# wusize/CLIPSelf

Measured on AMD Instinct MI355X. Metric: images/sec (student+teacher distill step), ViT-B/16 32 crops/img, higher is better.
Workload: dtype bf16; 1 GPU; EVA02-CLIP-B-16 CLIPSelf image-patches step, 64 images x 32 crops per GPU, 224^2 (BASELINE configs[1]); global_batch=64, crops_per_image=32, image_size=224, parallelism=dp1, teacher_chunk=2048, teacher_last_block=cls_query_only, teacher_schedule=one_batch_ahead_on_side_stream

## Files before the change

clipself_amd/csrc/attention.hip:

```cpp
#include <type_traits>
#include "cs_common.h"
#include <cstdlib>

namespace {

constexpr int HD = 64;
constexpr float LOG2E = 1.4426950408889634f;


#define Z16 (f32x16{0.f, 0.f, 0.f, 0.f, 0.f, 0.f, 0.f, 0.f, 0.f, 0.f, 0.f, 0.f, 0.f, 0.f, 0.f, 0.f})
__device__ __forceinline__ f32x16 zero16() {
    f32x16 z;
#pragma unroll
    for (int e = 0; e < 16; ++e) z[e] = 0.f;
    return z;
}

__device__ __forceinline__ void rope8(U128& v, const float* __restrict__ cs, const float* __restrict__ sn) {
    const float4 c0 = *(const float4*)cs, c1 = *(const float4*)(cs + 4);
    const float4 s0 = *(const float4*)sn, s1 = *(const float4*)(sn + 4);
    const float c[8] = {c0.x, c0.y, c0.z, c0.w, c1.x, c1.y, c1.z, c1.w};
    const float s[8] = {s0.x, s0.y, s0.z, s0.w, s1.x, s1.y, s1.z, s1.w};
#pragma unroll
    for (int j = 0; j < 4; ++j) {
        const float x0 = bf2f(v.e[2 * j]), x1 = bf2f(v.e[2 * j + 1]);
        v.e[2 * j] = f2bf(__builtin_fmaf(x0, c[2 * j], -(x1 * s[2 * j])));
        v.e[2 * j + 1] = f2bf(__builtin_fmaf(x1, c[2 * j + 1], x0 * s[2 * j + 1]));
    }
}

__device__ __forceinline__ void rope8_lds(U128& v, const float* rt, int g, float inv_g, int tok, int c8) {
    const int t = tok - 1;
    const int r = (int)(((float)t + 0.5f) * inv_g), c = t - r * g;
    const float* cs = rt + ((c8 < 4 ? r : 2 * g + c) << 5) + (c8 & 3) * 8;
    rope8(v, cs, cs + (g << 5));
}

template <int NT>
__device__ __forceinline__ void load_rope_tables(float* rt, const float* __restrict__ cos_t, const float* __restrict__ sin_t, int g, int tid) {
    for (int i = tid; i < g * 32; i += NT) {
        const int r = i >> 5, d = i & 31;
        rt[i] = cos_t[(size_t)(r * g) * HD + d];
        rt[(g << 5) + i] = sin_t[(size_t)(r * g) * HD + d];
        rt[(2 * g << 5) + i] = cos_t[(size_t)r * HD + 32 + d];
        rt[(3 * g << 5) + i] = sin_t[(size_t)r * HD + 32 + d];
    }
}

__device__ __forceinline__ bf16x8 pack8(const f32x16& a, int c2) {
    bf16x8 r;
#pragma unroll
    for (int j = 0; j < 8; ++j) r[j] = f2bf(a[c2 * 8 + j]);
    return r;
}

__device__ __forceinline__ bf16x8 load_t_frag(const __bf16* t, int ld, int d, int base, int hf) {
    U64 lo, hi;
    lo.u = *(const uint2*)(t + d * ld + base + 4 * hf);
    hi.u = *(const uint2*)(t + d * ld + base + 8 + 4 * hf);
    bf16x8 r;
#pragma unroll
    for (int j = 0; j < 4; ++j) { r[j] = lo.e[j]; r[4 + j] = hi.e[j]; }
    return r;
}

#ifdef CS_ABLATION_SWITCHES
#define ATT_ABL(p, bit) ((p).dbg & (bit))
#else
#define ATT_ABL(p, bit) false
#endif
struct AttnArgs {
    const __bf16* qkv;
    const __bf16* dout;
    const float* cos_t;
    const float* sin_t;
    const float* lse_in;
    const float* dsum;
    int dbg;
    int grid;
    float inv_grid;
    float* stats_part;
    long Mtot;
    __bf16* out;
    float* lse_out;
    int Ntok, H, ldqkv, ldo;
    float scale;
    int sch_on, sch_f0, sch_r, sch_bh, sch_fb, sch_rem, sch_absorb;
    const __bf16* qk;
    int ldqk;
};

struct RowBlock { int bh, tile0, nt; };
__device__ __forceinline__ RowBlock map_block(const AttnArgs& p, int waves) {
    RowBlock r;
    if (!p.sch_on) {
        r.bh = blockIdx.y; r.tile0 = blockIdx.x * waves; r.nt = waves;
        return r;
    }
    const int id = blockIdx.x;
    if (id < p.sch_f0) {
        const int qb = id / p.sch_bh;
        r.bh = id - qb * p.sch_bh; r.tile0 = qb * 8; r.nt = 8;
    } else if (id < p.sch_f0 + 2 * p.sch_r) {
        const int j = id - p.sch_f0, k = p.sch_f0 + (j >> 1), half = j & 1, qb = k / p.sch_bh;
        r.bh = k - qb * p.sch_bh; r.tile0 = qb * 8 + half * 4;
        r.nt = 4 + ((p.sch_absorb && half && qb == p.sch_fb - 1) ? p.sch_rem : 0);
    } else {
        r.bh = id - p.sch_f0 - 2 * p.sch_r; r.tile0 = p.sch_fb * 8; r.nt = p.sch_rem;
    }
    return r;
}

template <int CHK, bool ROPE, bool WITH_T>
__device__ __forceinline__ void stage_rows(const __bf16* __restrict__ src, size_t rowbase, int ld, int coloff, int tok0, int Ntok,
                                           const float* cos_t, const float* sin_t, char* tile, __bf16* tile_t, int ldt, int tid) {
    for (int idx = tid; idx < CHK * 8; idx += 512) {
        const int r = idx >> 3, c = idx & 7, tok = tok0 + r;
        U128 v;
        if (tok < Ntok) {
            v.u = *(const uint4*)(src + (rowbase + tok) * ld + coloff + c * 8);
            if (ROPE && tok > 0) rope8(v, cos_t + (size_t)(tok - 1) * HD + c * 8, sin_t + (size_t)(tok - 1) * HD + c * 8);
        } else {
            v.u = make_uint4(0, 0, 0, 0);
        }
        if (tile) *(uint4*)(tile + r * 128 + ((c ^ (r & 7)) << 4)) = v.u;
        if (WITH_T) {
#pragma unroll
            for (int e = 0; e < 8; ++e) tile_t[(c * 8 + e) * ldt + r] = v.e[e];
        }
    }
}

__device__ __forceinline__ bf16x8 lds_frag(const char* tile, int row, int ks, int hf) {
    return *(const bf16x8*)(tile + row * 128 + ((((ks << 1) + hf) ^ (row & 7)) << 4));
}

constexpr int VT_LD = 264;

__device__ __forceinline__ int k_off(int r, int c) { return ((r >> 1) << 8) + (((((r & 1) << 3) | c) ^ ((r >> 1) & 15)) << 4); }

typedef short s16x4v __attribute__((ext_vector_type(4)));

__device__ __forceinline__ int tr_lane_off(int rr, int d0, int lane) {
    const int li = lane & 15, g1 = (lane >> 4) & 1;
    const int col = d0 + 16 * g1 + 4 * (li & 3);
    return k_off(rr + (li >> 2), col >> 3) + ((col >> 2) & 1) * 8;
}
__device__ __forceinline__ bf16x8 tr_join2(s16x4v lo, s16x4v hi) {
    typedef short s16x8v __attribute__((ext_vector_type(8)));
    const s16x8v v = __builtin_shufflevector(lo, hi, 0, 1, 2, 3, 4, 5, 6, 7);
    return __builtin_bit_cast(bf16x8, v);
}
__device__ __forceinline__ s16x4v tr_read4(const char* addr) {
    return __builtin_amdgcn_ds_read_tr16_b64_v4i16((__attribute__((address_space(3))) s16x4v*)addr);
}

// ... 653 lines not shown
    {
        U128 t[4];
#pragma unroll
        for (int ks = 0; ks < 4; ++ks) {
            t[ks].u = PRE ? *(const uint4*)(p.qk + (rowbase + kc) * p.ldqk + C + h * HD + ks * 16 + hf * 8)
                          : *(const uint4*)(p.qkv + (rowbase + kc) * p.ldqkv + C + h * HD + ks * 16 + hf * 8);
            vf[ks] = *(const bf16x8*)(p.qkv + (rowbase + kc) * p.ldqkv + 2 * C + h * HD + ks * 16 + hf * 8);
        }
#pragma unroll
        for (int ks = 0; ks < 4; ++ks) {
            if (!PRE && ROPE && kc > 0) rope8_lds(t[ks], rt, p.grid, p.inv_grid, kc, ks * 2 + hf);
            kf[ks] = t[ks].h;
        }
    }
    f32x16 dk[2] = {zero16(), zero16()}, dv[2] = {zero16(), zero16()};
    const int k_base = (l31 >> 1) << 8, par8 = (l31 & 1) << 3, sw = l31 >> 1;
    int toff[2][2][2];
#pragma unroll
    for (int c2 = 0; c2 < 2; ++c2)
#pragma unroll
        for (int dt = 0; dt < 2; ++dt) {
            toff[c2][dt][0] = tr_lane_off(c2 * 16 + 4 * hf, dt * 32, lane);
            toff[c2][dt][1] = tr_lane_off(c2 * 16 + 8 + 4 * hf, dt * 32, lane);
        }

    for (int q0 = 0; q0 < (SINGLE ? 1 : p.Ntok); q0 += CHQ) {
        if (q0) __syncthreads();
        qr.template store<!PRE && ROPE>(Ql, rt, p.grid, p.inv_grid, q0, p.Ntok, tid);
        gr.template store<false>(Gl, rt, p.grid, p.inv_grid, q0, p.Ntok, tid);
        if (tid < CHQ) { lse_s[tid] = lse_r; dsum_s[tid] = dsum_r; }
        __syncthreads();
        if (!SINGLE && PF && q0 + CHQ < p.Ntok) {
            qr.load(qsrc, rowbase, qld, h * HD, q0 + CHQ, p.Ntok, tid);
            gr.load(p.dout, rowbase, p.ldo, h * HD, q0 + CHQ, p.Ntok, tid);
            load_stats(q0 + CHQ);
        }
        auto tile = [&](int t) {
            f32x16 s, dp;
#pragma unroll
            for (int ks = 0; ks < 4; ++ks) {
                const int off = t * (16 * 256) + k_base + (((par8 | (ks * 2 + hf)) ^ sw) << 4);
                s = __builtin_amdgcn_mfma_f32_32x32x16_bf16(*(const bf16x8*)(Ql + off), kf[ks], ks ? s : Z16, 0, 0, 0);
                dp = __builtin_amdgcn_mfma_f32_32x32x16_bf16(*(const bf16x8*)(Gl + off), vf[ks], ks ? dp : Z16, 0, 0, 0);
            }
#pragma unroll
            for (int k4 = 0; k4 < 4; ++k4) {
                const float4 l4 = *(const float4*)(lse_s + t * 32 + 8 * k4 + 4 * hf), d4 = *(const float4*)(dsum_s + t * 32 + 8 * k4 + 4 * hf);
                const float ls[4] = {l4.x, l4.y, l4.z, l4.w}, ds[4] = {d4.x, d4.y, d4.z, d4.w};
#pragma unroll
                for (int r = 0; r < 4; ++r) {
                    const int e = k4 * 4 + r;
                    const float pv = __builtin_amdgcn_exp2f(fmaf(s[e], sl2, -ls[r]));
                    s[e] = pv;
                    dp[e] = pv * fmaf(dp[e], p.scale, -ds[r]);
                }
            }
#pragma unroll
            for (int c2 = 0; c2 < 2; ++c2) {
                const bf16x8 pb = pack8(s, c2), db = pack8(dp, c2);
#pragma unroll
                for (int dt = 0; dt < 2; ++dt) {
                    const int o0 = t * (16 * 256) + toff[c2][dt][0], o1 = t * (16 * 256) + toff[c2][dt][1];
                    dv[dt] = __builtin_amdgcn_mfma_f32_32x32x16_bf16(tr_join2(tr_read4(Gl + o0), tr_read4(Gl + o1)), pb, dv[dt], 0, 0, 0);
                    dk[dt] = __builtin_amdgcn_mfma_f32_32x32x16_bf16(tr_join2(tr_read4(Ql + o0), tr_read4(Ql + o1)), db, dk[dt], 0, 0, 0);
                }
            }
        };
        if (wave_active) {
#pragma unroll
            for (int t = 0; t < CH; ++t) {
                if (q0 + t * 32 >= p.Ntok) break;
                tile(t);
            }
        }
    }
    if (wave_active && key < p.Ntok) {
        const size_t pos = (size_t)(key > 0 ? key - 1 : 0) * HD;
        __bf16* row = p.out + (rowbase + key) * p.ldqkv + h * HD;
        store_grad_tile(dk, row + C, ROPE && key > 0, p.cos_t + pos, p.sin_t + pos, hf);
        store_grad_tile(dv, row + 2 * C, false, nullptr, nullptr, hf);
    }
}

int att_num_cus() {
    static const int n = [] {
        int dev = 0, v = 0;
        if (hipGetDevice(&dev) != hipSuccess || hipDeviceGetAttribute(&v, hipDeviceAttributeMultiprocessorCount, dev) != hipSuccess || v <= 0) v = 256;
        return v;
    }();
    return n;
}
int set_schedule(AttnArgs& a, int B, int Ntok, int H, dim3& grid) {
    const int nt = (Ntok + 31) / 32, fb = nt / 8, rem = nt % 8, BH = B * H, F = fb * BH, G = att_num_cus();
    int R = F % G;
    if (getenv("CS_ATTN_NOSPLIT") || fb == 0 || 2 * R > G) R = 0;
    if (R == 0) {
        a.sch_on = 0;
        grid = dim3((Ntok + 255) / 256, BH);
        return 0;
    }
    a.sch_on = 1; a.sch_f0 = F - R; a.sch_r = R; a.sch_bh = BH; a.sch_fb = fb; a.sch_rem = rem;
    a.sch_absorb = rem > 0 && rem <= 4 && R >= BH;
    grid = dim3(F + R + ((rem > 0 && !a.sch_absorb) ? BH : 0), 1);
    return 1;
}

template <typename K>
void set_lds(K kernel, size_t bytes) { (void)hipFuncSetAttribute((const void*)kernel, hipFuncAttributeMaxDynamicSharedMemorySize, (int)bytes); }

int check_common(const char* who, int B, int Ntok, int H, int ldqkv, int ldo) {
    CS_CHECK_ARG(B > 0 && Ntok > 1 && H > 0, "%s: bad shape B=%d N=%d H=%d", who, B, Ntok, H);
    CS_CHECK_ARG(ldqkv % 8 == 0 && ldo % 8 == 0 && ldqkv >= 3 * H * HD && ldo >= H * HD, "%s: bad leading dimensions", who);
    return 0;
}

int check_tables(const char* who, const float* cos_t, const float* sin_t) {
    CS_CHECK_ARG((cos_t == nullptr) == (sin_t == nullptr), "%s: cos_t and sin_t are given together, or both NULL (no rotary embedding); got %s only",
                 who, cos_t ? "cos_t" : "sin_t");
    return 0;
}

template <int HG>
__global__ __launch_bounds__(256) void attn_cls_kernel(const __bf16* __restrict__ q, const __bf16* __restrict__ kv,
                                                       const float* __restrict__ cos_t, const float* __restrict__ sin_t,
                                                       __bf16* __restrict__ out, int Ntok, int H, int ldq, int ldkv, int ldo, float scale,
                                                       int qpb, const unsigned char* __restrict__ allow, float* __restrict__ lse_out) {
    extern __shared__ float sm[];
    const int Npad = (Ntok + 3) & ~3;
    float* rsum = sm + HG * Npad;
    float* part = rsum + 8;
    const int tid = threadIdx.x, lane = tid & 63, wave = tid >> 6;
    const int b = blockIdx.x, h0 = blockIdx.y * HG;
    const int c = tid & 7, kg = tid >> 3;
    const __bf16* kbase = kv + (size_t)(b / qpb) * Ntok * ldkv + h0 * HD + c * 8;
    const unsigned char* arow = allow ? allow + (size_t)b * Ntok : nullptr;
    const __bf16* vbase = kbase + H * HD;
    float qf[HG][8];
#pragma unroll
    for (int h = 0; h < HG; ++h) {
        U128 t;
        t.u = *(const uint4*)(q + (size_t)b * ldq + (h0 + h) * HD + c * 8);
#pragma unroll
        for (int j = 0; j < 8; ++j) qf[h][j] = bf2f(t.e[j]);
    }
    const float sl2 = scale * LOG2E;
    for (int key = kg; key < Ntok; key += 32) {
        U128 kk[HG];
#pragma unroll
        for (int h = 0; h < HG; ++h) kk[h].u = *(const uint4*)(kbase + (size_t)key * ldkv + h * HD);
        if (key > 0 && cos_t) {
            const float* cs = cos_t + (size_t)(key - 1) * HD + c * 8;
            const float* sn = sin_t + (size_t)(key - 1) * HD + c * 8;
#pragma unroll
            for (int h = 0; h < HG; ++h) rope8(kk[h], cs, sn);
        }
#pragma unroll
        for (int h = 0; h < HG; ++h) {
            float dot = 0.f;
#pragma unroll
            for (int j = 0; j < 8; ++j) dot += qf[h][j] * bf2f(kk[h].e[j]);
            dot += __shfl_xor(dot, 1);
            dot += __shfl_xor(dot, 2);
            dot += __shfl_xor(dot, 4);
            if (c == 0) sm[h * Npad + key] = (arow && !arow[key]) ? -INFINITY : dot * sl2;
        }
    }
    __syncthreads();
    for (int h = wave; h < HG; h += 4) {
        float* row = sm + h * Npad;
        float mx = -INFINITY;
        for (int key = lane; key < Ntok; key += 64) mx = fmaxf(mx, row[key]);
        mx = wave_max(mx);
        const bool no_key = mx == -INFINITY;
        if (no_key) mx = 0.f;
        float sum = 0.f;
        for (int key = lane; key < Ntok; key += 64) {
            const float e = __builtin_amdgcn_exp2f(row[key] - mx);
            sum += e;
            row[key] = bf2f(f2bf(e));
        }
        sum = wave_sum(sum);
        if (lane == 0) rsum[h] = sum > 0.f ? sum : 1.f;
        if (lane == 0 && lse_out)
            lse_out[((size_t)(b / qpb) * H + h0 + h) * qpb + b % qpb] = no_key ? INFINITY : (mx + __builtin_log2f(sum)) * (1.f / LOG2E);
    }
    __syncthreads();
    float acc[HG][8];
// ... 320 lines not shown
}

}

static int attn_fwd_impl(const void* qkv, const float* cos_t, const float* sin_t, void* out, float* lse, float* stats_part, int B, int Ntok,
                         int H, int ldqkv, int ldo, float scale, hipStream_t stream) {
    if (check_common("cs_attn_fwd", B, Ntok, H, ldqkv, ldo) || check_tables("cs_attn_fwd", cos_t, sin_t)) return -1;
    const bool rope = cos_t != nullptr;
    AttnArgs a{};
    a.qkv = (const __bf16*)qkv; a.cos_t = cos_t; a.sin_t = sin_t; a.out = (__bf16*)out; a.lse_out = lse;
    a.stats_part = stats_part; a.Mtot = (long)B * Ntok;
    int g = 0;
    if (rope) {
        g = (int)(sqrtf((float)(Ntok - 1)) + 0.5f);
        CS_CHECK_ARG(g * g == Ntok - 1, "cs_attn_fwd: Ntok - 1 = %d is not a square token grid (the RoPE tables are read separably)", Ntok - 1);
        a.grid = g; a.inv_grid = 1.f / (float)g;
    }
#ifdef CS_ABLATION_SWITCHES
    static const int dbg_env = getenv("CS_ATTN_DBG") ? atoi(getenv("CS_ATTN_DBG")) : 0;
    a.dbg = dbg_env;
#else
    a.dbg = 0;
#endif
    a.Ntok = Ntok; a.H = H; a.ldqkv = ldqkv; a.ldo = ldo; a.scale = scale;
    constexpr int CH = 7;
    const size_t lds = (size_t)CH * 32 * 128 + (size_t)HD * VT_LD * 2 + (size_t)4 * g * 32 * sizeof(float);
    CS_CHECK_ARG(lds <= 160 * 1024, "cs_attn_fwd: token grid %d too large for the LDS RoPE tables", g);
    if (Ntok <= CH * 32) {
        static bool once = (set_lds(attn_fwd8_kernel<false>, 160 * 1024), set_lds(attn_fwd8_kernel<true>, 160 * 1024),
                            set_lds(attn_fwd8_kernel<false, false>, 160 * 1024), set_lds(attn_fwd8_kernel<true, false>, 160 * 1024), true);
        (void)once;
        const bool tail = Ntok > (CH - 1) * 32;
        if (rope) {
            if (tail) hipLaunchKernelGGL((attn_fwd8_kernel<true>), dim3(1, B * H), dim3(512), lds, stream, a);
            else hipLaunchKernelGGL((attn_fwd8_kernel<false>), dim3(1, B * H), dim3(512), lds, stream, a);
        } else {
            if (tail) hipLaunchKernelGGL((attn_fwd8_kernel<true, false>), dim3(1, B * H), dim3(512), lds, stream, a);
            else hipLaunchKernelGGL((attn_fwd8_kernel<false, false>), dim3(1, B * H), dim3(512), lds, stream, a);
        }
    } else {
        static bool once = (set_lds(attn_fwd2_kernel<CH, 4>, 160 * 1024), set_lds(attn_fwd2_kernel<CH, 4, false>, 160 * 1024), true);
        (void)once;
        const size_t lds2 = (size_t)2 * CH * 32 * 128 + (size_t)4 * g * 32 * sizeof(float);
        dim3 grid2;
        set_schedule(a, B, Ntok, H, grid2);
        if (rope) hipLaunchKernelGGL((attn_fwd2_kernel<CH, 4>), grid2, dim3(512), lds2, stream, a);
        else hipLaunchKernelGGL((attn_fwd2_kernel<CH, 4, false>), grid2, dim3(512), lds2, stream, a);
    }
    CS_LAUNCH_CHECK();
    return 0;
}

extern "C" int cs_attn_fwd(const void* qkv, const float* cos_t, const float* sin_t, void* out, float* lse, int B, int Ntok, int H,
                           int ldqkv, int ldo, float scale, hipStream_t stream) {
    return attn_fwd_impl(qkv, cos_t, sin_t, out, lse, nullptr, B, Ntok, H, ldqkv, ldo, scale, stream);
}

extern "C" int cs_attn_fwd_stats(const void* qkv, const float* cos_t, const float* sin_t, void* out, float* lse, float* stats_part, int B,
                                 int Ntok, int H, int ldqkv, int ldo, float scale, hipStream_t stream) {
    CS_CHECK_ARG(stats_part != nullptr && ((uintptr_t)stats_part % 8) == 0, "cs_attn_fwd_stats: stats_part must be an 8-byte aligned buffer");
    return attn_fwd_impl(qkv, cos_t, sin_t, out, lse, stats_part, B, Ntok, H, ldqkv, ldo, scale, stream);
}

static size_t bwd_dsum_bytes(int B, int Ntok, int H) { return (((size_t)B * H * Ntok * sizeof(float)) + 255) & ~(size_t)255; }
static size_t bwd_image_bytes(int B, int Ntok, int H) {
    return bwd_dsum_bytes(B, Ntok, H) + (Ntok > 7 * 32 ? (size_t)B * Ntok * 2 * H * HD * sizeof(__bf16) : 0);
}
extern "C" size_t cs_attn_bwd_workspace(int B, int Ntok, int H, int Q) {
    const size_t img = bwd_image_bytes(B, Ntok, H);
    if (Q <= 0) return img;
    return ((img + 255) & ~(size_t)255) + (size_t)B * H * ((Ntok + PKB - 1) / PKB) * Q * HD * sizeof(float);
}

struct cs_attn_extra {
    const void* q;
    const void* o;
    const void* dout;
    const float* lse;
    const unsigned char* allow;
    void* dq;
    int Q, ldq, ldo, lddq;
};

static int attn_bwd_image(const void* qkv, const void* o, const void* dout, const float* lse, const float* cos_t, const float* sin_t,
                          void* dqkv, void* workspace, int B, int Ntok, int H, int ldqkv, int ldo, float scale, hipStream_t stream) {
    CS_CHECK_ARG(workspace != nullptr && lse != nullptr, "cs_attn_bwd: workspace and lse are required");
    float* dsum = (float*)workspace;
    const long total = (long)B * Ntok * H * 8;
    hipLaunchKernelGGL(attn_bwd_prep_kernel, dim3((int)((total + 255) / 256)), dim3(256), 0, stream, (const __bf16*)o, (const __bf16*)dout, dsum, B, Ntok, H, ldo);
    CS_LAUNCH_CHECK();
    AttnArgs a{};
    a.qkv = (const __bf16*)qkv; a.dout = (const __bf16*)dout; a.cos_t = cos_t; a.sin_t = sin_t; a.lse_in = lse; a.dsum = dsum;
    a.out = (__bf16*)dqkv; a.Ntok = Ntok; a.H = H; a.ldqkv = ldqkv; a.ldo = ldo; a.scale = scale;
    dim3 grid((Ntok + 255) / 256, B * H), block(512);
    constexpr int CH = 7;
    constexpr int CHK = CH * 32, VLD = CHK + 4;
    const bool tables = cos_t != nullptr;
    const int g = tables ? (int)(sqrtf((float)(Ntok - 1)) + 0.5f) : 0;
    const bool v1 = tables && (getenv("CS_ATTN_BWD_V1") != nullptr || g * g != Ntok - 1);
    if (!v1) {
        a.grid = g; a.inv_grid = tables ? 1.f / (float)g : 0.f;
        const size_t rope = (size_t)4 * g * 32 * sizeof(float);
        const size_t lds_dq = (size_t)2 * CHK * 128 + rope, lds_dkv = (size_t)2 * CHK * 128 + (size_t)2 * CHK * sizeof(float) + rope;
        CS_CHECK_ARG(lds_dkv <= 160 * 1024, "cs_attn_bwd: token grid %d too large for the LDS RoPE tables", g);
        static bool once = (set_lds(attn_bwd_dq2_kernel<CH, true>, 160 * 1024), set_lds(attn_bwd_dkv2_kernel<CH, true>, 160 * 1024),
                            set_lds(attn_bwd_dq2_kernel<CH, false, true>, 160 * 1024), set_lds(attn_bwd_dkv2_kernel<CH, false, true>, 160 * 1024),
                            set_lds(attn_bwd_dq2_kernel<CH, true, false, false>, 160 * 1024), set_lds(attn_bwd_dkv2_kernel<CH, true, false, false>, 160 * 1024),
                            set_lds(attn_bwd_dq2_kernel<CH, false, true, false>, 160 * 1024), set_lds(attn_bwd_dkv2_kernel<CH, false, true, false>, 160 * 1024),
                            true);
        (void)once;
        if (!tables) {
            if (Ntok <= CHK) {
                hipLaunchKernelGGL((attn_bwd_dq2_kernel<CH, true, false, false>), grid, block, lds_dq, stream, a);
                CS_LAUNCH_CHECK();
                hipLaunchKernelGGL((attn_bwd_dkv2_kernel<CH, true, false, false>), grid, block, lds_dkv, stream, a);
            } else {
                dim3 grid2;
                set_schedule(a, B, Ntok, H, grid2);
                a.qk = (const __bf16*)qkv; a.ldqk = ldqkv;
                hipLaunchKernelGGL((attn_bwd_dq2_kernel<CH, false, true, false>), grid2, block, lds_dq, stream, a);
                CS_LAUNCH_CHECK();
                hipLaunchKernelGGL((attn_bwd_dkv2_kernel<CH, false, true, false>), grid2, block, lds_dkv, stream, a);
            }
        } else if (Ntok <= CHK) {
            hipLaunchKernelGGL((attn_bwd_dq2_kernel<CH, true>), grid, block, lds_dq, stream, a);
            CS_LAUNCH_CHECK();
            hipLaunchKernelGGL((attn_bwd_dkv2_kernel<CH, true>), grid, block, lds_dkv, stream, a);
        } else {
            dim3 grid2;
            set_schedule(a, B, Ntok, H, grid2);
            const int C2 = 2 * H * HD;
            __bf16* qk = (__bf16*)((char*)workspace + bwd_dsum_bytes(B, Ntok, H));
            const long items = (long)B * Ntok * (C2 / 8);
            hipLaunchKernelGGL(rope_qk_kernel, dim3((unsigned)((items + 255) / 256)), dim3(256), 0, stream, (const __bf16*)qkv, cos_t, sin_t, qk,
                               (long)B * Ntok, Ntok, H * HD, ldqkv);
            CS_LAUNCH_CHECK();
            a.qk = qk; a.ldqk = C2;
            hipLaunchKernelGGL((attn_bwd_dq2_kernel<CH, false, true>), grid2, block, lds_dq - rope, stream, a);
            CS_LAUNCH_CHECK();
            hipLaunchKernelGGL((attn_bwd_dkv2_kernel<CH, false, true>), grid2, block, lds_dkv - rope, stream, a);
        }
        CS_LAUNCH_CHECK();
        return 0;
    }
    const size_t lds_dq = (size_t)2 * CHK * 128 + (size_t)HD * VLD * 2;
    const size_t lds_dkv = (size_t)2 * CHK * 128 + (size_t)2 * HD * VLD * 2 + (size_t)2 * CHK * sizeof(float);
    static bool once = (set_lds(attn_bwd_dq_kernel<CH>, lds_dq), set_lds(attn_bwd_dkv_kernel<CH>, lds_dkv), true);
    (void)once;
    hipLaunchKernelGGL((attn_bwd_dq_kernel<CH>), grid, block, lds_dq, stream, a);
    CS_LAUNCH_CHECK();
    hipLaunchKernelGGL((attn_bwd_dkv_kernel<CH>), grid, block, lds_dkv, stream, a);
    CS_LAUNCH_CHECK();
    return 0;
}

extern "C" int cs_attn_bwd(const void* qkv, const void* o, const void* dout, const float* lse, const float* cos_t, const float* sin_t,
                           void* dqkv, void* workspace, int B, int Ntok, int H, int ldqkv, int ldo, float scale, const cs_attn_extra* extra,
                           hipStream_t stream) {
    if (check_common("cs_attn_bwd", B, Ntok, H, ldqkv, ldo) || check_tables("cs_attn_bwd", cos_t, sin_t)) return -1;
    if (extra == nullptr) return attn_bwd_image(qkv, o, dout, lse, cos_t, sin_t, dqkv, workspace, B, Ntok, H, ldqkv, ldo, scale, stream);
    const cs_attn_extra& e = *extra;
    const bool image = o != nullptr || dout != nullptr || lse != nullptr;
    CS_CHECK_ARG(qkv && dqkv && workspace, "cs_attn_bwd: qkv, dqkv and workspace are required");
    CS_CHECK_ARG(!image || (o && dout && lse), "cs_attn_bwd: with extra rows, o / dout / lse of the image rows are given together or not at all");
    CS_CHECK_ARG(e.q && e.o && e.dout && e.lse && e.allow && e.dq && e.Q > 0, "cs_attn_bwd: extra rows: null pointer or Q=%d", e.Q);
    CS_CHECK_ARG(e.ldq % 8 == 0 && e.ldo % 8 == 0 && e.lddq % 8 == 0 && e.ldq >= H * HD && e.ldo >= H * HD && e.lddq >= H * HD,
                 "cs_attn_bwd: extra rows: row strides must be multiples of 8 and cover the heads (ldq=%d ldo=%d lddq=%d)", e.ldq, e.ldo, e.lddq);
    CS_CHECK_ARG(((uintptr_t)e.q % 16) == 0 && ((uintptr_t)e.o % 16) == 0 && ((uintptr_t)e.dout % 16) == 0 && ((uintptr_t)e.dq % 16) == 0 &&
                 ((uintptr_t)qkv % 16) == 0 && ((uintptr_t)dqkv % 16) == 0, "cs_attn_bwd: extra rows: buffers must be 16-byte aligned");
    if (image && attn_bwd_image(qkv, o, dout, lse, cos_t, sin_t, dqkv, workspace, B, Ntok, H, ldqkv, ldo, scale, stream)) return -1;
    PassArgs p{};
    p.qkv = (const __bf16*)qkv; p.q = (const __bf16*)e.q; p.o = (const __bf16*)e.o; p.dout = (const __bf16*)e.dout; p.lse = e.lse;
    p.allow = e.allow; p.dqkv = (__bf16*)dqkv; p.dq = (__bf16*)e.dq;
    p.part = (float*)((char*)workspace + ((bwd_image_bytes(B, Ntok, H) + 255) & ~(size_t)255));
    p.Ntok = Ntok; p.H = H; p.Q = e.Q; p.ldqkv = ldqkv; p.ldq = e.ldq; p.ldo = e.ldo; p.lddq = e.lddq;
    p.nkb = (Ntok + PKB - 1) / PKB; p.assign = image ? 0 : 1; p.scale = scale;
    hipLaunchKernelGGL(attn_pass_bwd_kernel, dim3(p.nkb, B * H), dim3(256), 0, stream, p);
    CS_LAUNCH_CHECK();
    const long total = (long)B * H * e.Q * 8;
    hipLaunchKernelGGL(attn_pass_dq_kernel, dim3((unsigned)((total + 255) / 256)), dim3(256), 0, stream, p, total);
    CS_LAUNCH_CHECK();
    return 0;
}

static int attn_cls_launch(const void* q, const void* kv, const float* cos_t, const float* sin_t, void* out, int rows, int Ntok, int H,
                           int ldq, int ldkv, int ldo, float scale, int qpb, const unsigned char* allow, float* lse, hipStream_t stream) {
    const int HG = H % 6 == 0 ? 6 : (H % 4 == 0 ? 4 : (H % 3 == 0 ? 3 : (H % 2 == 0 ? 2 : 1)));
// ... 75 lines not shown
```

clipself_amd/hip.py:

```python
from __future__ import annotations

import ctypes
import os
import subprocess
from pathlib import Path

import torch

_CSRC = Path(__file__).resolve().parent / "csrc"
_LIB_PATH = Path(os.environ["CLIPSELF_HIP_LIB"]) if os.environ.get("CLIPSELF_HIP_LIB") else _CSRC / "libclipself_hip.so"

EPI_BF16, EPI_F32, EPI_RESID_F32, EPI_SWIGLU_BF16, EPI_ATOMIC_F32, EPI_PATCH_F32, EPI_RESID_LN_F32, EPI_GELU_BF16, EPI_QGELU_BF16 = range(9)
DX_BF16, DX_F32_ASSIGN, DX_F32_ACCUM = range(3)
ADAMW_GUARD_HEAD, ADAMW_GUARD_SPAN = 8, 16384

_vp, _i, _l, _f, _sz = ctypes.c_void_p, ctypes.c_int, ctypes.c_long, ctypes.c_float, ctypes.c_size_t

SIGNATURES = {
    "cs_last_error": (ctypes.c_char_p, []),
    "cs_gemm_nt": (_i, [_vp, _vp, _vp, _vp, _vp, _i, _i, _i, _i, _i, _i, _i, _i, _i, _i, _vp]),
    "cs_crop_resize_workspace": (_sz, [_i, _i, _i]),
    "cs_crop_resize_u8": (_i, [_vp, _i, _i, _vp, _i, _i, _i, _vp, _vp, _vp, _vp, _vp]),
    "cs_quant_rows_fp8": (_i, [_vp, _l, _vp, _l, _vp, _i, _i, _vp]),
    "cs_gemm_nt_f8": (_i, [_vp, _vp, _vp, _vp, _vp, _vp, _vp, _i, _i, _i, _i, _i, _i, _i, _i, _vp]),
    "cs_resize_bilinear_f32": (_i, [_vp, _vp, _i, _i, _i, _i, _i, _vp]),
    "cs_gemm_wgrad_workspace": (_sz, [_i, _i, _i]),
    "cs_gemm_wgrad": (_i, [_vp, _vp, _vp, _vp, _i, _i, _i, _i, _i, _i, _vp]),
    "cs_gemm_wgrad_tn_workspace": (_sz, [_i, _i, _i]),
    "cs_gemm_wgrad_tn": (_i, [_vp, _vp, _vp, _vp, _i, _i, _i, _i, _i, _i, _vp]),
    "cs_gemm_nt_ln": (_i, [_vp, _vp, _vp, _vp, _vp, _vp, _vp, _vp, _vp, _vp, _i, _i, _i, _i, _i, _i, _i, _i, _i, _i, _i, _vp]),
    "cs_gemm_nt_ln_split": (_i, [_vp, _vp, _vp, _vp, _vp, _vp, _vp, _vp, _vp, _vp, _i, _vp, _i, _i, _i, _i, _i, _i, _i, _vp]),
    "cs_ln_stats_finalize": (_i, [_vp, _i, _i, _i, _i, _f, _vp, _vp, _vp]),
    "cs_attn_fwd_stats": (_i, [_vp, _vp, _vp, _vp, _vp, _vp, _i, _i, _i, _i, _i, _f, _vp]),
    "cs_layernorm_fwd": (_i, [_vp, _i, _l, _vp, _vp, _vp, _l, _vp, _vp, _i, _i, _f, _vp]),
    "cs_layernorm_fwd_q8": (_i, [_vp, _i, _l, _vp, _vp, _vp, _l, _vp, _vp, _vp, _l, _vp, _i, _i, _f, _vp]),
    "cs_layernorm_fwd_f32": (_i, [_vp, _l, _vp, _vp, _vp, _l, _vp, _vp, _i, _i, _f, _vp]),
    "cs_layernorm_bwd_workspace": (_sz, [_i, _i]),
    "cs_layernorm_bwd": (_i, [_vp, _l, _vp, _i, _l, _vp, _vp, _vp, _vp, _i, _l, _vp, _vp, _i, _vp, _vp, _l, _vp, _i, _i, _vp]),
    "cs_layernorm_bwd_q8": (_i, [_vp, _l, _vp, _i, _l, _vp, _vp, _vp, _vp, _i, _l, _vp, _vp, _i, _vp, _vp, _l, _vp, _vp, _l, _vp, _i, _i, _vp]),
    "cs_l2norm_fwd": (_i, [_vp, _vp, _vp, _i, _i, _f, _vp]),
    "cs_l2norm_bwd": (_i, [_vp, _vp, _vp, _vp, _i, _i, _vp]),
    "cs_attn_fwd": (_i, [_vp, _vp, _vp, _vp, _vp, _i, _i, _i, _i, _i, _f, _vp]),
    "cs_attn_cls_fwd": (_i, [_vp, _vp, _vp, _vp, _vp, _i, _i, _i, _i, _i, _i, _f, _vp]),
    "cs_attn_query_fwd": (_i, [_vp, _vp, _vp, _vp, _vp, _i, _i, _i, _i, _i, _i, _i, _f, _vp]),
    "cs_attn_bwd_workspace": (_sz, [_i, _i, _i, _i]),
    "cs_attn_bwd": (_i, [_vp, _vp, _vp, _vp, _vp, _vp, _vp, _vp, _i, _i, _i, _i, _i, _f, _vp, _vp]),
    "cs_swiglu_fwd": (_i, [_vp, _l, _vp, _l, _i, _i, _vp]),
    "cs_swiglu_bwd": (_i, [_vp, _l, _vp, _l, _vp, _l, _i, _i, _vp]),
    "cs_swiglu_bwd_colsum": (_i, [_vp, _l, _vp, _l, _vp, _l, _vp, _vp, _i, _i, _vp]),
    "cs_swiglu_bwd_q8": (_i, [_vp, _l, _vp, _l, _vp, _l, _vp, _l, _vp, _i, _i, _vp]),
    "cs_gelu_fwd": (_i, [_vp, _l, _vp, _l, _i, _i, _i, _vp]),
    "cs_gelu_bwd": (_i, [_vp, _l, _vp, _l, _vp, _l, _i, _i, _i, _vp]),
    "cs_cast_f32_bf16": (_i, [_vp, _vp, _l, _vp]),
    "cs_transpose_bf16": (_i, [_vp, _l, _vp, _l, _i, _i, _vp]),
    "cs_transpose_bf16_batched": (_i, [_vp, _i, _i, _vp]),
    "cs_colsum_workspace": (_sz, [_i, _i]),
    "cs_colsum_bf16": (_i, [_vp, _l, _vp, _vp, _i, _i, _vp]),
    "cs_im2row": (_i, [_vp, _i, _vp, _i, _i, _i, _i, _vp]),
    "cs_cls_row": (_i, [_vp, _vp, _vp, _i, _i, _i, _vp]),
    "cs_roialign_fwd": (_i, [_vp, _vp, _vp, _i, _i, _i, _i, _i, _i, _vp]),
    "cs_roialign_bwd": (_i, [_vp, _vp, _vp, _i, _i, _i, _i, _i, _i, _i, _vp]),
    "cs_cosine_loss_fwd": (_i, [_vp, _vp, _vp, _vp, _i, _i, _f, _vp]),
    "cs_cosine_loss_bwd": (_i, [_vp, _vp, _vp, _vp, _i, _i, _f, _f, _vp, _vp]),
    "cs_fed_bce_fwd": (_i, [_vp, _l, _vp, _vp, _vp, _i, _i, _f, _f, _vp]),
    "cs_fed_bce_bwd": (_i, [_vp, _l, _vp, _vp, _l, _i, _i, _f, _f, _vp, _vp]),
    "cs_num_compute_units": (_i, []),
    "cs_stream_create_cu_mask": (_i, [_i, _i, ctypes.POINTER(_vp)]),
    "cs_stream_destroy": (_i, [_vp]),
    "cs_adamw_step": (_i, [_vp, _vp, _vp, _vp, _vp, _vp, _l, _f, _f, _f, _f, _f, _i, _f, _f, _i, _vp, _vp]),
}


class AttnExtra(ctypes.Structure):
    _fields_ = [("q", _vp), ("o", _vp), ("dout", _vp), ("lse", _vp), ("allow", _vp), ("dq", _vp), ("Q", _i), ("ldq", _i), ("ldo", _i), ("lddq", _i)]


def library_path() -> Path:
    return _LIB_PATH


def build_library(force: bool = False) -> Path:
    if force:
        for o in _CSRC.glob("_obj_*.o"):
            o.unlink()
    subprocess.run(["bash", str(_CSRC / "build.sh")], check=True)
    return _LIB_PATH


_lib = None


def load_library():
    global _lib
    if _lib is None:
        if not _LIB_PATH.exists():
            raise RuntimeError(
                f"{_LIB_PATH} is missing: build it with clipself_amd/csrc/build.sh (or __graft_entry__.build()). "
                "There is no CPU fallback for the CLIPSelf hot path.")
        lib = ctypes.CDLL(str(_LIB_PATH))
        for name, (res, args) in SIGNATURES.items():
            fn = getattr(lib, name)
            fn.restype, fn.argtypes = res, args
        _lib = lib
    return _lib


def _p(t):
    return None if t is None else t.data_ptr()


def _dt(t) -> int:
    if t.dtype == torch.float32:
        return 0
    if t.dtype == torch.bfloat16:
        return 1
    raise TypeError(f"unsupported dtype {t.dtype}")


def _readable(t, n) -> bool:
    return t is None or t.untyped_storage().nbytes() - t.storage_offset() * t.element_size() >= n * t.element_size()


class HipOps:

    name = "hip"
    ATTN_EXTRA_QUERIES = True
    ATTN_CAUSAL = True
    ADAMW_GUARD = True
    ATTN_NO_ROPE = True

    def __init__(self):
        self.lib = load_library()
        if not torch.cuda.is_available():
            raise RuntimeError("HipOps needs a ROCm device (torch.cuda.is_available() is False); no CPU fallback exists")
        self.gemm_flags = 0
        self._rccl_reserve = 0
        self._share = 0
        self._cap = 0
        self.num_cus = int(self.lib.cs_num_compute_units())

    def _update_flags(self):
        n = self._rccl_reserve + self._share
        if self._cap:
            n = max(n, self.num_cus - self._cap)
        if not (0 <= n <= self.num_cus - 8 and n < 256):
            raise ValueError(f"persistent GEMM grids keep at least 8 workgroups and can leave at most 255 compute units free "
                             f"(asked to leave {n} of {self.num_cus} CUs: RCCL reserve {self._rccl_reserve}, tower share {self._share}, cap {self._cap})")
        self.gemm_flags = (self.gemm_flags & ~(255 << 20)) | (int(n) << 20)

    def reserve_compute_units(self, n: int):
        self._rccl_reserve = int(n)
        self._update_flags()

    def share_compute_units(self, n: int):
        self._share = int(n)
        self._update_flags()

    def cap_compute_units(self, n: int):
        self._cap = int(n)
        self._update_flags()

    def persistent_grid(self) -> int:
        return self.num_cus - ((self.gemm_flags >> 20) & 255)

    def num_compute_units(self) -> int:
        return self.num_cus

    def stream_create_cu_mask(self, first_cu: int, n_cus: int):
        h = ctypes.c_void_p()
        self._ok(self.lib.cs_stream_create_cu_mask(int(first_cu), int(n_cus), ctypes.byref(h)), "cs_stream_create_cu_mask")
        s = torch.cuda.ExternalStream(h.value)
# ... 453 lines not shown
```

Measured before the change: 749.6 images/sec.

## Fuse attention backward prep, dK/dV and dQ into one per-head kernel

Adds a single attention-backward kernel for sequences up to 224 tokens, with one workgroup per (batch, head). It computes the dO·O row sums in-kernel and keeps dS in LDS so dQ is computed from it directly. This replaces the separate prep, dQ and dKV launches, which recomputed S and P twice and round-tripped dsum through global memory. The cost is a large LDS footprint per block, which may reduce occupancy, and only B*H workgroups per launch. The fused path becomes the default, and an env switch falls back to the old path.

```diff
diff --git a/clipself_amd/csrc/attention.hip b/clipself_amd/csrc/attention.hip
--- a/clipself_amd/csrc/attention.hip
+++ b/clipself_amd/csrc/attention.hip
@@ -72,6 +72,7 @@
 struct AttnArgs {
     const __bf16* qkv;
     const __bf16* dout;
+    const __bf16* o;
     const float* cos_t;
     const float* sin_t;
     const float* lse_in;
@@ -891,6 +892,211 @@
     }
 }
 
+constexpr int FUSED_ROWS = 224, FUSED_DS_LD = 464;
+
+__device__ __forceinline__ void store_grad_tile_rows(const f32x16 (&g)[2], char* slab, bool rope, const float* cs_lo, const float* cs_hi, int sn_off,
+                                                     __bf16* dst, int ld, int tok0, int Ntok, int lane) {
+    const int hf = lane >> 5, l31 = lane & 31;
+#pragma unroll
+    for (int dt = 0; dt < 2; ++dt)
+#pragma unroll
+        for (int g4 = 0; g4 < 4; ++g4) {
+            float v[4] = {g[dt][g4 * 4], g[dt][g4 * 4 + 1], g[dt][g4 * 4 + 2], g[dt][g4 * 4 + 3]};
+            if (rope) {
+                const float* cs = (dt ? cs_hi : cs_lo) + g4 * 8 + hf * 4;
+                const float4 c = *(const float4*)cs, s = *(const float4*)(cs + sn_off);
+                const float a0 = __builtin_fmaf(v[0], c.x, v[1] * s.y), a1 = __builtin_fmaf(v[1], c.y, -(v[0] * s.x));
+                const float a2 = __builtin_fmaf(v[2], c.z, v[3] * s.w), a3 = __builtin_fmaf(v[3], c.w, -(v[2] * s.z));
+                v[0] = a0; v[1] = a1; v[2] = a2; v[3] = a3;
+            }
+            U64 t;
+#pragma unroll
+            for (int i = 0; i < 4; ++i) t.e[i] = f2bf(v[i]);
+            *(uint2*)(slab + l31 * 128 + (((dt * 4 + g4) ^ (l31 & 7)) << 4) + hf * 8) = t.u;
+        }
+    asm volatile("s_waitcnt lgkmcnt(0)" ::: "memory");
+#pragma unroll
+    for (int i = 0; i < 4; ++i) {
+        const int r = i * 8 + (lane >> 3), c = lane & 7;
+        const uint4 v = *(const uint4*)(slab + r * 128 + ((c ^ (r & 7)) << 4));
+        if (tok0 + r < Ntok) *(uint4*)(dst + (size_t)(tok0 + r) * ld + c * 8) = v;
+    }
+    asm volatile("s_waitcnt lgkmcnt(0)" ::: "memory");
+}
+template <bool ROPE>
+__global__ __launch_bounds__(512, 2) void attn_bwd_fused_kernel(AttnArgs p) {
+    constexpr int CH = FUSED_ROWS / 32, NT = 512, ITEMS = (FUSED_ROWS * 8 + NT - 1) / NT;
+    extern __shared__ __attribute__((aligned(16))) char smem[];
+    const int nt = (p.Ntok + 31) >> 5;
+    char* Ql = smem;
+    char* Gl = smem + nt * 4096;
+    float* lse_s = (float*)(smem + 2 * nt * 4096);
+    float* dsum_s = lse_s + FUSED_ROWS;
+    float* rt = dsum_s + FUSED_ROWS;
+    char* Sl = (char*)(rt + (ROPE ? 4 * p.grid * 32 : 0));
+
+    const int tid = threadIdx.x, lane = tid & 63, wave = tid >> 6, hf = lane >> 5, l31 = lane & 31;
+    const int bh = blockIdx.x, b = bh / p.H, h = bh - b * p.H;
+    const int C = p.H * HD;
+    const size_t rowbase = (size_t)b * p.Ntok;
+    const int key = wave * 32 + l31;
+    const int kc = min(key, p.Ntok - 1);
+    const bool wave_active = wave < nt;
+    const float sl2 = p.scale * LOG2E;
+
+    uint4 qv[ITEMS], gv[ITEMS], ov[ITEMS];
+#pragma unroll
+    for (int it = 0; it < ITEMS; ++it) {
+        const int idx = tid + it * NT, tok = min(idx >> 3, p.Ntok - 1), c = idx & 7;
+        qv[it] = *(const uint4*)(p.qkv + (rowbase + tok) * p.ldqkv + h * HD + c * 8);
+        gv[it] = *(const uint4*)(p.dout + (rowbase + tok) * p.ldo + h * HD + c * 8);
+        ov[it] = *(const uint4*)(p.o + (rowbase + tok) * p.ldo + h * HD + c * 8);
+    }
+    float lse_r = INFINITY;
+    if (tid < p.Ntok) lse_r = p.lse_in[(size_t)bh * p.Ntok + tid] * LOG2E;
+    bf16x8 kf[4], vf[4];
+    U128 kt4[4];
+#pragma unroll
+    for (int ks = 0; ks < 4; ++ks) {
+        kt4[ks].u = *(const uint4*)(p.qkv + (rowbase + kc) * p.ldqkv + C + h * HD + ks * 16 + hf * 8);
+        vf[ks] = *(const bf16x8*)(p.qkv + (rowbase + kc) * p.ldqkv + 2 * C + h * HD + ks * 16 + hf * 8);
+    }
+    if constexpr (ROPE) {
+        load_rope_tables<NT>(rt, p.cos_t, p.sin_t, p.grid, tid);
+        __syncthreads();
+    }
+#pragma unroll
+    for (int ks = 0; ks < 4; ++ks) {
+        if (ROPE && kc > 0) rope8_lds(kt4[ks], rt, p.grid, p.inv_grid, kc, ks * 2 + hf);
+        kf[ks] = kt4[ks].h;
+    }
+#pragma unroll
+    for (int it = 0; it < ITEMS; ++it) {
+        const int idx = tid + it * NT, r = idx >> 3, c = idx & 7;
+        U128 a, g;
+        a.u = ov[it];
+        g.u = gv[it];
+        float s = 0.f;
+#pragma unroll
+        for (int e = 0; e < 8; ++e) s += bf2f(a.e[e]) * bf2f(g.e[e]);
+        s = sum_lanes8(s);
+        if (idx < nt * 256) {
+            U128 t;
+            t.u = qv[it];
+            if (ROPE && r > 0 && r < p.Ntok) rope8_lds(t, rt, p.grid, p.inv_grid, r, c);
+            *(uint4*)(Ql + k_off(r, c)) = t.u;
+            *(uint4*)(Gl + k_off(r, c)) = g.u;
+            if (c == 0) dsum_s[r] = r < p.Ntok ? s * p.scale : 0.f;
+        }
+    }
+    if (tid < nt * 32) lse_s[tid] = lse_r;
+    __syncthreads();
+
+    const int k_base = (l31 >> 1) << 8, par8 = (l31 & 1) << 3, sw = l31 >> 1;
+    int toff[2][2][2];
+#pragma unroll
+    for (int c2 = 0; c2 < 2; ++c2)
+#pragma unroll
+        for (int dt = 0; dt < 2; ++dt) {
+            toff[c2][dt][0] = tr_lane_off(c2 * 16 + 4 * hf, dt * 32, lane);
+            toff[c2][dt][1] = tr_lane_off(c2 * 16 + 8 + 4 * hf, dt * 32, lane);
+        }
+
+    f32x16 dk[2] = {zero16(), zero16()}, dv[2] = {zero16(), zero16()};
+    if (wave_active) {
+        const bool kpad = key >= p.Ntok;
+        char* srow = Sl + (4 * hf) * FUSED_DS_LD + key * 2;
+        auto tile = [&](int t) {
+            f32x16 s, dp;
+#pragma unroll
+            for (int ks = 0; ks < 4; ++ks) {
+                const int off = t * (16 * 256) + k_base + (((par8 | (ks * 2 + hf)) ^ sw) << 4);
+                s = __builtin_amdgcn_mfma_f32_32x32x16_bf16(*(const bf16x8*)(Ql + off), kf[ks], ks ? s : Z16, 0, 0, 0);
+                dp = __builtin_amdgcn_mfma_f32_32x32x16_bf16(*(const bf16x8*)(Gl + off), vf[ks], ks ? dp : Z16, 0, 0, 0);
+            }
+#pragma unroll
+            for (int k4 = 0; k4 < 4; ++k4) {
+                const float4 l4 = *(const float4*)(lse_s + t * 32 + 8 * k4 + 4 * hf), d4 = *(const float4*)(dsum_s + t * 32 + 8 * k4 + 4 * hf);
+                const float ls[4] = {l4.x, l4.y, l4.z, l4.w}, ds[4] = {d4.x, d4.y, d4.z, d4.w};
+#pragma unroll
+                for (int r = 0; r < 4; ++r) {
+                    const int e = k4 * 4 + r;
+                    const float pv = __builtin_amdgcn_exp2f(fmaf(s[e], sl2, -ls[r]));
+                    s[e] = pv;
+                    dp[e] = pv * fmaf(dp[e], p.scale, -ds[r]);
+                }
+            }
+            bf16x8 pb[2], db[2];
+#pragma unroll
+            for (int c2 = 0; c2 < 2; ++c2) { pb[c2] = pack8(s, c2); db[c2] = pack8(dp, c2); }
+            if (t * 32 + 32 <= p.Ntok) {
+#pragma unroll
+                for (int e = 0; e < 16; ++e)
+                    *(__bf16*)(srow + (t * 32 + (e & 3) + 8 * (e >> 2)) * FUSED_DS_LD) = kpad ? f2bf(0.f) : db[e >> 3][e & 7];
+            } else {
+#pragma unroll
+                for (int e = 0; e < 16; ++e)
+                    if (t * 32 + mfma32_row(e, lane) < p.Ntok)
+                        *(__bf16*)(srow + (t * 32 + (e & 3) + 8 * (e >> 2)) * FUSED_DS_LD) = kpad ? f2bf(0.f) : db[e >> 3][e & 7];
+            }
+#pragma unroll
+            for (int c2 = 0; c2 < 2; ++c2)
+#pragma unroll
+                for (int dt = 0; dt < 2; ++dt) {
+                    const int o0 = t * (16 * 256) + toff[c2][dt][0], o1 = t * (16 * 256) + toff[c2][dt][1];
+                    dv[dt] = __builtin_amdgcn_mfma_f32_32x32x16_bf16(tr_join2(tr_read4(Gl + o0), tr_read4(Gl + o1)), pb[c2], dv[dt], 0, 0, 0);
+                    dk[dt] = __builtin_amdgcn_mfma_f32_32x32x16_bf16(tr_join2(tr_read4(Ql + o0), tr_read4(Ql + o1)), db[c2], dk[dt], 0, 0, 0);
+                }
+        };
+#pragma unroll
+        for (int t = 0; t < CH; ++t) {
+            if (t * 32 >= p.Ntok) break;
+            tile(t);
+        }
+    }
+    __syncthreads();
+    char* slab = Ql + wave * 4096;
+    const float *cs_lo = rt, *cs_hi = rt;
+    const int sn_off = p.grid << 5;
+    if (ROPE && kc > 0) {
+        const int tm = kc - 1, r = (int)(((float)tm + 0.5f) * p.inv_grid), c = tm - r * p.grid;
+        cs_lo = rt + (r << 5);
+        cs_hi = rt + ((2 * p.grid + c) << 5);
+    }
+    __bf16* const out_h = p.out + rowbase * p.ldqkv + h * HD;
+    if (wave_active) {
+#pragma unroll
+        for (int ks = 0; ks < 4; ++ks) *(bf16x8*)(Gl + k_off(key, ks * 2 + hf)) = kf[ks];
+        store_grad_tile_rows(dv, slab, false, cs_lo, cs_hi, sn_off, out_h + 2 * C, p.ldqkv, wave * 32, p.Ntok, lane);
+        store_grad_tile_rows(dk, slab, ROPE && kc > 0, cs_lo, cs_hi, sn_off, out_h + C, p.ldqkv, wave * 32, p.Ntok, lane);
+    }
+    __syncthreads();
+
+    if (wave_active) {
+        f32x16 dq[2] = {zero16(), zero16()};
+        const char* srow = Sl + kc * FUSED_DS_LD + (4 * hf) * 2;
+#pragma unroll
+        for (int t = 0; t < CH; ++t) {
+            if (t * 32 >= p.Ntok) break;
+#pragma unroll
+            for (int c2 = 0; c2 < 2; ++c2) {
+                U64 lo, hi;
+                lo.u = *(const uint2*)(srow + (t * 32 + c2 * 16) * 2);
+                hi.u = *(const uint2*)(srow + (t * 32 + c2 * 16 + 8) * 2);
+                bf16x8 db;
+#pragma unroll
+                for (int j = 0; j < 4; ++j) { db[j] = lo.e[j]; db[4 + j] = hi.e[j]; }
+#pragma unroll
+                for (int dt = 0; dt < 2; ++dt) {
+                    const bf16x8 kt = tr_join2(tr_read4(Gl + t * (16 * 256) + toff[c2][dt][0]), tr_read4(Gl + t * (16 * 256) + toff[c2][dt][1]));
+                    dq[dt] = __builtin_amdgcn_mfma_f32_32x32x16_bf16(kt, db, dq[dt], 0, 0, 0);
+                }
+            }
+        }
+        store_grad_tile_rows(dq, slab, ROPE && kc > 0, cs_lo, cs_hi, sn_off, out_h, p.ldqkv, wave * 32, p.Ntok, lane);
+    }
+}
+
 int att_num_cus() {
     static const int n = [] {
         int dev = 0, v = 0;
@@ -912,6 +1118,11 @@
     a.sch_absorb = rem > 0 && rem <= 4 && R >= BH;
     grid = dim3(F + R + ((rem > 0 && !a.sch_absorb) ? BH : 0), 1);
     return 1;
+}
+
+bool getenv_flag(const char* name) {
+    const char* v = getenv(name);
+    return v && v[0] && v[0] != '0';
 }
 
 template <typename K>
@@ -1398,27 +1609,55 @@
     int Q, ldq, ldo, lddq;
 };
 
+enum BwdForm { BWD_V1, BWD_FUSED, BWD_SINGLE, BWD_CHUNKED };
+static BwdForm bwd_form(int Ntok, bool tables, int g) {
+    if (tables && (getenv("CS_ATTN_BWD_V1") != nullptr || g * g != Ntok - 1)) return BWD_V1;
+    if (Ntok > FUSED_ROWS) return BWD_CHUNKED;
+    const char* sw = getenv("CLIPSELF_ATTN_BWD_FUSED");
+    return sw && sw[0] == '0' ? BWD_SINGLE : BWD_FUSED;
+}
+static size_t fused_lds_bytes(int Ntok, int g) {
+    const size_t nt = (size_t)(Ntok + 31) / 32;
+    return 2 * nt * 4096 + 2 * FUSED_ROWS * sizeof(float) + (size_t)4 * g * 32 * sizeof(float) + (size_t)Ntok * FUSED_DS_LD;
+}
+
 static int attn_bwd_image(const void* qkv, const void* o, const void* dout, const float* lse, const float* cos_t, const float* sin_t,
                           void* dqkv, void* workspace, int B, int Ntok, int H, int ldqkv, int ldo, float scale, hipStream_t stream) {
     CS_CHECK_ARG(workspace != nullptr && lse != nullptr, "cs_attn_bwd: workspace and lse are required");
+    const bool tables = cos_t != nullptr;
+    const int g = tables ? (int)(sqrtf((float)(Ntok - 1)) + 0.5f) : 0;
+    const BwdForm form = bwd_form(Ntok, tables, g);
     float* dsum = (float*)workspace;
-    const long total = (long)B * Ntok * H * 8;
-    hipLaunchKernelGGL(attn_bwd_prep_kernel, dim3((int)((total + 255) / 256)), dim3(256), 0, stream, (const __bf16*)o, (const __bf16*)dout, dsum, B, Ntok, H, ldo);
-    CS_LAUNCH_CHECK();
+    if (form != BWD_FUSED) {
+        const long total = (long)B * Ntok * H * 8;
+        hipLaunchKernelGGL(attn_bwd_prep_kernel, dim3((int)((total + 255) / 256)), dim3(256), 0, stream, (const __bf16*)o, (const __bf16*)dout, dsum, B, Ntok, H, ldo);
+        CS_LAUNCH_CHECK();
+    }
     AttnArgs a{};
-    a.qkv = (const __bf16*)qkv; a.dout = (const __bf16*)dout; a.cos_t = cos_t; a.sin_t = sin_t; a.lse_in = lse; a.dsum = dsum;
+    a.qkv = (const __bf16*)qkv; a.dout = (const __bf16*)dout; a.o = (const __bf16*)o; a.cos_t = cos_t; a.sin_t = sin_t; a.lse_in = lse; a.dsum = dsum;
     a.out = (__bf16*)dqkv; a.Ntok = Ntok; a.H = H; a.ldqkv = ldqkv; a.ldo = ldo; a.scale = scale;
     dim3 grid((Ntok + 255) / 256, B * H), block(512);
     constexpr int CH = 7;
     constexpr int CHK = CH * 32, VLD = CHK + 4;
-    const bool tables = cos_t != nullptr;
-    const int g = tables ? (int)(sqrtf((float)(Ntok - 1)) + 0.5f) : 0;
-    const bool v1 = tables && (getenv("CS_ATTN_BWD_V1") != nullptr || g * g != Ntok - 1);
-    if (!v1) {
+    if (getenv_flag("CS_ATTN_DEBUG"))
+        fprintf(stderr, "cs_attn_bwd: form=%s B=%d Ntok=%d H=%d tables=%d fused_lds=%zu\n",
+                form == BWD_FUSED ? "fused" : (form == BWD_SINGLE ? "single" : (form == BWD_CHUNKED ? "chunked" : "v1")), B, Ntok, H, (int)tables,
+                form == BWD_FUSED ? fused_lds_bytes(Ntok, g) : (size_t)0);
+    if (form != BWD_V1) {
         a.grid = g; a.inv_grid = tables ? 1.f / (float)g : 0.f;
         const size_t rope = (size_t)4 * g * 32 * sizeof(float);
         const size_t lds_dq = (size_t)2 * CHK * 128 + rope, lds_dkv = (size_t)2 * CHK * 128 + (size_t)2 * CHK * sizeof(float) + rope;
         CS_CHECK_ARG(lds_dkv <= 160 * 1024, "cs_attn_bwd: token grid %d too large for the LDS RoPE tables", g);
+        if (form == BWD_FUSED) {
+            static bool once_f = (set_lds(attn_bwd_fused_kernel<true>, 160 * 1024), set_lds(attn_bwd_fused_kernel<false>, 160 * 1024), true);
+            (void)once_f;
+            const size_t lds = fused_lds_bytes(Ntok, g);
+            CS_CHECK_ARG(((uintptr_t)dqkv % 16) == 0, "cs_attn_bwd: dqkv must be 16-byte aligned (whole 128-byte rows are stored)");
+            if (tables) hipLaunchKernelGGL((attn_bwd_fused_kernel<true>), dim3(B * H), block, lds, stream, a);
+            else hipLaunchKernelGGL((attn_bwd_fused_kernel<false>), dim3(B * H), block, lds, stream, a);
+            CS_LAUNCH_CHECK();
+            return 0;
+        }
         static bool once = (set_lds(attn_bwd_dq2_kernel<CH, true>, 160 * 1024), set_lds(attn_bwd_dkv2_kernel<CH, true>, 160 * 1024),
                             set_lds(attn_bwd_dq2_kernel<CH, false, true>, 160 * 1024), set_lds(attn_bwd_dkv2_kernel<CH, false, true>, 160 * 1024),
                             set_lds(attn_bwd_dq2_kernel<CH, true, false, false>, 160 * 1024), set_lds(attn_bwd_dkv2_kernel<CH, true, false, false>, 160 * 1024),
diff --git a/clipself_amd/hip.py b/clipself_amd/hip.py
--- a/clipself_amd/hip.py
+++ b/clipself_amd/hip.py
@@ -87,6 +87,26 @@
     return _LIB_PATH
 
 
+ATTN_BWD_FUSED_ROWS = 224
+ATTN_BWD_FUSED_DS_LD = 464
+
+
+def attn_bwd_form(Ntok: int, tables: bool, fused_switch=None, v1_switch=None) -> str:
+    fused_switch = os.environ.get("CLIPSELF_ATTN_BWD_FUSED") if fused_switch is None else fused_switch
+    v1_switch = os.environ.get("CS_ATTN_BWD_V1") if v1_switch is None else v1_switch
+    g = int((Ntok - 1) ** 0.5 + 0.5)
+    if tables and (v1_switch is not None or g * g != Ntok - 1):
+        return "v1"
+    if Ntok > ATTN_BWD_FUSED_ROWS:
+        return "chunked"
+    return "single" if fused_switch is not None and fused_switch[:1] == "0" else "fused"
+
+
+def attn_bwd_fused_lds_bytes(Ntok: int, grid: int = 0) -> int:
+    nt = (Ntok + 31) // 32
+    return 2 * nt * 4096 + 2 * ATTN_BWD_FUSED_ROWS * 4 + 4 * grid * 32 * 4 + Ntok * ATTN_BWD_FUSED_DS_LD
+
+
 _lib = None
 
 
```

After: 754.2 images/sec, median of 6. No clear change (+0.6%).
